# atenpas/gpd

Measured on AMD Instinct MI355X. Metric: 15-ch grasp candidates scored/sec (imagegen+LeNet) at 1/2/4/8 MI355X, higher is better.
Workload: dtype f64 geometry / u8 images / LeNet f32-equivalent by exact operand splitting: conv1 int8 digit planes of 32-bit fixed-point weights (i32 accumulate, exact), conv2 + ip1 three bf16 pieces per operand (six exact products per term, f32 accumulate), ip2 f32

## Files before the change

gpd_amd/csrc/gpd_internal.h:

```cpp
#pragma once
#include <hip/hip_runtime.h>
#include <stdint.h>

#include <cmath>

#include <vector>

#ifdef GPD_PROFILING
#include <cstdlib>
#include <rocprofiler-sdk-roctx/roctx.h>
#endif

#include "../../include/gpd_hip.h"

namespace gpd {

constexpr int kImg = 60;
constexpr int kPix = kImg * kImg;
constexpr int kFc1In = 7200;
constexpr int kFc1Out = 500;
__host__ __device__ inline size_t fc1p_index(int m, int kq, int u) { return (((size_t)(m >> 5) * 4 + kq) * kFc1Out + u) * 32 + (m & 31); }
constexpr int kLenetXld = 7296;

struct LeNetFast {
// ... 297 lines not shown
                 gpd_hand *d_out, hipStream_t stream);
int gather_records(const gpd_hand *d_all, const int32_t *d_sel, int k, gpd_hand *d_out, hipStream_t stream);
int select_topk_capacity();

struct ImageState {
  unsigned long long lcg_base = 0;
  int num_candidates = 0;
  int capacity = 0;
  uint8_t *d_images = nullptr;
  uint8_t *d_images_hwc = nullptr;
  uint32_t *d_set_bits = nullptr;
  int num_shadow_sets = 0, cap_shadow_sets = 0;
  bool wide = false;
  bool huge = false;
  int set_sd = 0, set_sr = 0;
  size_t cap_setwords = 0;
  int32_t *d_overflow2 = nullptr;
  char *d_huge_scratch = nullptr;
  int channels = 0;
  int slots = 0;
  int32_t *d_overflow = nullptr;
  int32_t *d_pts_overflow = nullptr;
  char *d_pts_scratch = nullptr;
  int32_t *d_status = nullptr;
  long long stat_sets = 0, stat_sum_set_ni = 0, stat_sum_cand_ni = 0;
  std::vector<unsigned char> consts;
  double view_points[3 * kMaxCams] = {0};
  hipStream_t aux = nullptr;
  hipEvent_t ev_fork = nullptr, ev_join = nullptr;
  bool side_stream = true;
};
int images_reserve(const gpd_params &p, ImageState &im, int n, int shadow_sets);
int images_run(const gpd_params &p, const Cloud &c, const SearchState &s, const Plan &pl, ImageState &im, hipStream_t stream);
int images_launch(const SearchState &s, const Plan &pl, ImageState &im, hipStream_t stream, bool counters_clean = false);
void images_status_text(int status, char *buf, size_t len);
int images_routes(const ImageState &im, int32_t *route, long long info[8]);
hipError_t planar_to_hwc(const uint8_t *src, uint8_t *dst, int n, int C, hipStream_t stream);
hipError_t hwc_to_planar(const uint8_t *src, uint8_t *dst, int n, int C, hipStream_t stream);
void image_cell_thresholds(double len, double *out);
void images_free(ImageState &im);

struct HostConsts {
  double rot[GPD_MAX_SLOTS][9];
  double rot_binormal[9];
  double finger_spacing[32];
  double deepen_depths[128];
// ... 46 lines not shown
```

gpd_amd/csrc/images.hip:

```cpp
#include <cfloat>
#include <cmath>
#include <cstddef>
#include <cstdio>
#include <cstdlib>
#include <cstring>

#include <mutex>
#include <type_traits>

#include "gpd_internal.h"

namespace gpd {

#define HIP_RET(expr)                                                                       \
  do {                                                                                      \
    hipError_t e_ = (expr);                                                                 \
    if (e_ != hipSuccess) {                                                                 \
      set_error("%s failed: %s (%s:%d)", #expr, hipGetErrorString(e_), __FILE__, __LINE__); \
      return GPD_ERR_HIP;                                                                   \
    }                                                                                       \
  } while (0)

constexpr int IMG_THREADS = 512;
constexpr int SET_THREADS = 1024;
// ... 3 lines not shown
constexpr int SH_CAP = 6144;
constexpr int SH_CAP_BIG = 12288;
template <bool WIDE>
struct Vox {
  static constexpr int VD = WIDE ? 64 : 46;
  static constexpr int SD = WIDE ? 128 : 86;
  static constexpr int SR = WIDE ? 64 : 43;
  static constexpr int LB = 18;
  static constexpr int SETWORDS = (SD * SD * SD + 31) / 32;
};

struct ImgConsts {
  double vol_depth, vol_width, vol_height, half_od, dbl_h;
  int C, nproj, per;
  double shadow_length, voxel, voxel_mult, rand_inv;
  int num_shadow;
  uint32_t stride_a, stride_c;
  double len[3];
  double inv_cell[3];
  double thr[3][kImg + 1];
  double inv_len[3];
  int true_div;
  int set_sd, set_sr;
};
__constant__ ImgConsts c_img;

struct ImgParams {
  const float *nn;
  int cap;
  const double *centers;
  const gpd_hand *hands;
  const int32_t *cand_hand;
  const int32_t *meta;
  const uint32_t *set_bits;
  uint8_t *images;
  int32_t *status;
  int num_cand;
  const int32_t *cand_list;
  const int32_t *cand_count;
  int32_t *overflow_list;
  int32_t *overflow_count;
  unsigned long long *dbg;
  int32_t *pts_overflow_list;
  int32_t *pts_overflow_count;
  char *pts_scratch;
  int exit_after;
  char *huge_scratch;
};

struct Box {
  double F[9];
  double sample[3];
  double off[3];
  double lo[3], hi[3];
};

constexpr size_t PTS_SCRATCH_BYTES = (size_t)PT_CAP_BIG * (3 * sizeof(double) + sizeof(float4) + sizeof(uint32_t));
struct PointArrays {
  double t[3][PT_CAP];
  float4 an[PT_CAP];
};
struct NoPointArrays {};
template <bool BIG>
struct __attribute__((aligned(16))) SmemPts {
  typename std::conditional<BIG, NoPointArrays, PointArrays>::type p;
  __attribute__((aligned(16))) uint32_t cells[kPix];
  uint16_t place[BIG ? PT_CAP_BIG : PT_CAP];
  float4 nzv[(BIG ? kPix : PT_CAP) + 1];
  uint16_t nzlist[BIG ? kPix : PT_CAP];
  double thr[3][kImg + 1];
  double recip[128];
  float red_f[4 * IMG_WAVES];
  int red_i[IMG_WAVES];
  int counter;
  int flag;
  int nnz;
};
typedef SmemPts<false> Smem;
template <int SHC, bool WIDE>
struct __attribute__((aligned(16))) SmemShadow {
  __attribute__((aligned(16))) float raster0[kPix];
  __attribute__((aligned(16))) uint32_t cells[kPix];
  uint32_t lin[SHC];
  union {
    struct {
      uint16_t rowbase[Vox<WIDE>::VD * Vox<WIDE>::VD];
      uint8_t rowcnt[Vox<WIDE>::VD * Vox<WIDE>::VD];
    } rows;
    uint16_t place[SHC];
  } bp;
  uint16_t nz[kPix];
  uint8_t cz[SHC];
  double thr[3][kImg + 1];
  double recip[128];
  float red_f[4 * IMG_WAVES];
  int red_i[IMG_WAVES];
  int vorg[3];
  int flag;
  int nnz;
};

__device__ inline double uniform_f64(double v) {
  const unsigned long long b = (unsigned long long)__double_as_longlong(v);
  const unsigned lo = __builtin_amdgcn_readfirstlane((unsigned)b);
  const unsigned hi = __builtin_amdgcn_readfirstlane((unsigned)(b >> 32));
  return __longlong_as_double((long long)(((unsigned long long)hi << 32) | lo));
}

template <class OP>
__device__ inline float wave_reduce_f32(float v, OP op) {
  auto dpp = [](float x, auto ctrl, auto rmask) {
    return __int_as_float(__builtin_amdgcn_update_dpp(__float_as_int(x), __float_as_int(x), decltype(ctrl)::value, decltype(rmask)::value, 0xf, false));
  };
  using std::integral_constant;
  v = op(v, dpp(v, integral_constant<int, 0xB1>(), integral_constant<int, 0xf>()));
  v = op(v, dpp(v, integral_constant<int, 0x4E>(), integral_constant<int, 0xf>()));
  v = op(v, dpp(v, integral_constant<int, 0x141>(), integral_constant<int, 0xf>()));
  v = op(v, dpp(v, integral_constant<int, 0x140>(), integral_constant<int, 0xf>()));
  v = op(v, dpp(v, integral_constant<int, 0x142>(), integral_constant<int, 0xa>()));
  v = op(v, dpp(v, integral_constant<int, 0x143>(), integral_constant<int, 0xc>()));
  return __int_as_float(__builtin_amdgcn_readlane(__float_as_int(v), 63));
}
__device__ inline float wave_max_f32(float v) { return wave_reduce_f32(v, [](float a, float b) { return fmaxf(a, b); }); }
__device__ inline float wave_min_f32(float v) { return wave_reduce_f32(v, [](float a, float b) { return fminf(a, b); }); }

__device__ inline int wave_incl_scan_i32(int v) {
  v += __builtin_amdgcn_update_dpp(0, v, 0x111, 0xf, 0xf, false);
  v += __builtin_amdgcn_update_dpp(0, v, 0x112, 0xf, 0xf, false);
  v += __builtin_amdgcn_update_dpp(0, v, 0x114, 0xf, 0xf, false);
  v += __builtin_amdgcn_update_dpp(0, v, 0x118, 0xf, 0xf, false);
// ... 457 lines not shown
#pragma unroll
      for (int i = 0; i < N; i++) {
        const int j = i ^ stride;
        if (j > i) {
          const uint32_t lo = min(k[i], k[j]), hi = max(k[i], k[j]);
          const bool up = (i & size) == 0;
          k[i] = up ? lo : hi;
          k[j] = up ? hi : lo;
        }
      }
    }
  }
}
template <int N>
__device__ inline void sort_u16_regs(uint16_t *p, int n) {
  uint32_t k[N];
#pragma unroll
  for (int q = 0; q < N; q++) k[q] = q < n ? (uint32_t)p[q] : 0xffffffffu;
  sort_regs<N>(k);
#pragma unroll
  for (int q = 0; q < N; q++)
    if (q < n) p[q] = (uint16_t)k[q];
}
#define TICK(k)                                                     \
  do {                                                              \
    if (P.dbg && tid == 0) {                                        \
      const unsigned long long now_ = __builtin_readcyclecounter(); \
      atomicAdd(&P.dbg[k], now_ - t_last);                          \
      t_last = now_;                                                \
    }                                                               \
  } while (0)

__device__ inline void load_box(const gpd_hand &H, Box &B) {
  const ImgConsts &K = c_img;
#pragma unroll
  for (int i = 0; i < 9; i++) B.F[i] = uniform_f64(H.frame[i]);
#pragma unroll
  for (int i = 0; i < 3; i++) B.sample[i] = uniform_f64(H.sample[i]);
  const double hb = uniform_f64(H.bottom), hc = uniform_f64(H.center);
  B.off[0] = hb;
  B.off[1] = uniform_f64(hc - K.half_od);
  B.off[2] = uniform_f64(-K.vol_height);
  B.lo[0] = hb;
  B.hi[0] = uniform_f64(hb + K.vol_depth);
  B.lo[1] = B.off[1];
  B.hi[1] = uniform_f64(hc + K.half_od);
  B.lo[2] = uniform_f64(-1.0 * K.vol_height);
  B.hi[2] = uniform_f64(K.vol_height);
}

__device__ __forceinline__ int xcd_candidate(int n) {
  const int per = (n + 7) >> 3;
  const int L = blockIdx.x, slot = L >> 3;
  const int cand = (L & 7) * per + slot;
  return cand < n ? cand : -1;
}

template <int SHC, bool WIDE>
__device__ __forceinline__ void shadow_image_body(const ImgParams &P, SmemShadow<SHC, WIDE> &S, const int cand) {
  constexpr int VDIM = Vox<WIDE>::VD, SD = Vox<WIDE>::SD, SR = Vox<WIDE>::SR, LB = Vox<WIDE>::LB, SETWORDS = Vox<WIDE>::SETWORDS;
  unsigned long long t_last = __builtin_readcyclecounter();
  const ImgConsts &K = c_img;
  const int tid = threadIdx.x;
  const int lane = tid & 63;
  const int set_ord = P.meta[4 * cand + 2];
  const int set_nb = P.meta[4 * cand + 3];
  uint8_t *out = P.images + (size_t)cand * kPix * K.C;
  Box B;
  load_box(P.hands[P.cand_hand[cand]], B);
  for (int i = tid; i < 3 * (kImg + 1); i += IMG_THREADS) (&S.thr[0][0])[i] = (&K.thr[0][0])[i];
  for (int i = tid; i < 128; i += IMG_THREADS) S.recip[i] = i ? 1.0 / (double)i : 0.0;
  for (int c = tid; c < kPix / 4; c += IMG_THREADS) reinterpret_cast<uint4 *>(S.cells)[c] = make_uint4(0u, 0u, 0u, 0u);
  if (tid == 0) {
    S.flag = 0;
    double lo[3] = {DBL_MAX, DBL_MAX, DBL_MAX}, hi[3] = {-DBL_MAX, -DBL_MAX, -DBL_MAX};
#pragma unroll
    for (int k = 0; k < 8; k++) {
      const double bx = (k & 1) ? B.hi[0] : B.lo[0];
      const double by = (k & 2) ? B.hi[1] : B.lo[1];
      const double bz = (k & 4) ? B.hi[2] : B.lo[2];
#pragma unroll
      for (int a = 0; a < 3; a++) {
        const double w = B.sample[a] + B.F[3 * a] * bx + B.F[3 * a + 1] * by + B.F[3 * a + 2] * bz;
        lo[a] = fmin(lo[a], w);
        hi[a] = fmax(hi[a], w);
      }
    }
    int bad = 0;
#pragma unroll
    for (int a = 0; a < 3; a++) {
      const int v0 = (int)floor(lo[a] * K.voxel_mult) - 1, v1 = (int)floor(hi[a] * K.voxel_mult) + 1;
      const int o = (int)floor(B.sample[a] * K.voxel_mult) - SR;
      S.vorg[a] = v0;
      if (v1 - v0 >= VDIM || v0 + 1 < o || v1 - 1 >= o + SD) bad = 1;
    }
    S.flag = bad;
  }
  __syncthreads();
  const int x0 = S.vorg[0], y0 = S.vorg[1], z0 = S.vorg[2];
  constexpr int NROWS = VDIM * VDIM, RPT = (NROWS + IMG_THREADS - 1) / IMG_THREADS;
  unsigned long long mask[RPT];
#pragma unroll
  for (int k = 0; k < RPT; k++) mask[k] = 0ull;
  if (set_ord >= 0) {
    const uint32_t *sb = P.set_bits + (size_t)set_ord * SETWORDS;
    const int ox = (int)floor(B.sample[0] * K.voxel_mult) - SR, oy = (int)floor(B.sample[1] * K.voxel_mult) - SR,
              oz = (int)floor(B.sample[2] * K.voxel_mult) - SR;
    const int zlo = z0 - oz;
    double invBz[3];
#pragma unroll
    for (int a = 0; a < 3; a++) {
      const double bz = B.F[6 + a] * K.voxel;
      invBz[a] = uniform_f64(fabs(bz) > 1e-9 ? 1.0 / bz : 0.0);
    }
    const int za = zlo < 0 ? 0 : zlo, zb = (zlo + VDIM < SD) ? zlo + VDIM : SD;
    const int nbits = zb - za;
    double T0[3], Ax[3], Ay[3], Lf[3], Wd[3];
    {
      const double wx = (double)x0 * K.voxel - B.sample[0], wy = (double)y0 * K.voxel - B.sample[1],
                   wz = (double)(za - zlo + z0) * K.voxel - B.sample[2];
#pragma unroll
      for (int a = 0; a < 3; a++) {
        T0[a] = uniform_f64(B.F[a] * wx + B.F[3 + a] * wy + B.F[6 + a] * wz);
        Ax[a] = uniform_f64(B.F[a] * K.voxel);
        Ay[a] = uniform_f64(B.F[3 + a] * K.voxel);
        Lf[a] = invBz[a] > 0.0 ? B.lo[a] : B.hi[a];
        Wd[a] = uniform_f64(fabs((B.hi[a] - B.lo[a]) * invBz[a]));
      }
    }
    unsigned long long fld[RPT];
#pragma unroll
    for (int k = 0; k < RPT; k++) fld[k] = 0ull;
    for (int cb = 0; cb < set_nb; cb++) {
      const uint32_t *sc = sb + (size_t)cb * SETWORDS;
      uint32_t wa[RPT], wb[RPT], wc[RPT];
#pragma unroll
      for (int k = 0; k < RPT; k++) {
        const int row = tid + k * IMG_THREADS;
        const int ix = row / VDIM, iy = row - ix * VDIM;
        const int sx = x0 + ix - ox, sy = y0 + iy - oy;
        const bool ok = row < NROWS && (unsigned)sx < (unsigned)SD && (unsigned)sy < (unsigned)SD && za < zb;
        const int w0 = ok ? ((sx * SD + sy) * SD + za) >> 5 : 0;
        wa[k] = sc[w0];
        wb[k] = sc[w0 + 1 < SETWORDS ? w0 + 1 : SETWORDS - 1];
        wc[k] = sc[w0 + 2 < SETWORDS ? w0 + 2 : SETWORDS - 1];
      }
#pragma unroll
      for (int k = 0; k < RPT; k++) {
        const int row = tid + k * IMG_THREADS;
        const int ix = row / VDIM, iy = row - ix * VDIM;
        const int sx = x0 + ix - ox, sy = y0 + iy - oy;
// ... 7 lines not shown
      }
    }
#pragma unroll
    for (int k = 0; k < RPT; k++) {
      const int row = tid + k * IMG_THREADS;
      if (row >= NROWS) continue;
      const int ix = row / VDIM, iy = row - ix * VDIM;
      unsigned long long field = fld[k];
      field &= (nbits >= 64) ? ~0ull : ((1ull << (nbits > 0 ? nbits : 0)) - 1ull);
      if (field) {
        constexpr double EPS = 1e-3;
        const double fx = (double)ix, fy = (double)iy;
        double dmin = 0.0, dmax = (double)(nbits - 1);
        double smin = 0.0, smax = (double)(nbits - 1);
#pragma unroll
        for (int a = 0; a < 3; a++) {
          const double tba = T0[a] + fx * Ax[a] + fy * Ay[a];
          if (invBz[a] != 0.0) {
            const double dl = (Lf[a] - tba) * invBz[a], dh = dl + Wd[a];
            dmin = fmax(dmin, dl - EPS);
            dmax = fmin(dmax, dh + EPS);
            smin = fmax(smin, dl + EPS);
            smax = fmin(smax, dh - EPS);
          } else if (tba < B.lo[a] - 1e-6 || tba > B.hi[a] + 1e-6) {
            dmax = -1.0;
          } else if (!(tba > B.lo[a] + 1e-6 && tba < B.hi[a] - 1e-6)) {
            smax = -1.0;
          }
        }
        if (dmax < dmin) {
          field = 0ull;
        } else {
          const int t0 = (int)ceil(dmin), t1 = (int)floor(dmax);
          if (t0 > 0) field &= ~((1ull << t0) - 1ull);
          if (t1 < 63) field &= (2ull << t1) - 1ull;
          if (smax >= smin) {
            const int u0 = (int)ceil(smin), u1 = (int)floor(smax);
            if (u1 >= u0) {
              unsigned long long sure = field;
              if (u0 > 0) sure &= ~((1ull << u0) - 1ull);
              if (u1 < 63) sure &= (2ull << u1) - 1ull;
              mask[k] |= sure << (za - zlo);
              field &= ~sure;
            }
          }
        }
      }
      while (field) {
        const int t = __ffsll((long long)field) - 1;
        field &= field - 1;
        const int iz = za + t - zlo;
        double th[3];
        to_hand(B, (double)(ix + x0) * K.voxel, (double)(iy + y0) * K.voxel, (double)(iz + z0) * K.voxel, th);
        if (in_box(B, th)) mask[k] |= 1ull << iz;
      }
    }
  }
#pragma unroll
  for (int k = 0; k < RPT; k++) {
    const int row = tid + k * IMG_THREADS;
    if (row < NROWS) S.bp.rows.rowcnt[row] = (uint8_t)__popcll(mask[k]);
  }
  __syncthreads();
  TICK(0);
  int cnt = 0;
#pragma unroll
  for (int k = 0; k < RPT; k++) {
    const int row = tid * RPT + k;
    if (row < NROWS) cnt += S.bp.rows.rowcnt[row];
  }
  int n_sh;
  int pos = block_excl_scan(S, cnt, &n_sh);
  if (n_sh > SHC) {
    if (tid == 0) {
      if (P.overflow_list) {
        const int slot = atomicAdd(P.overflow_count, 1);
        P.overflow_list[slot] = cand;
// ... 12 lines not shown
    }
  }
  __syncthreads();
#pragma unroll
  for (int k = 0; k < RPT; k++) {
    const int row = tid + k * IMG_THREADS;
    if (row >= NROWS) continue;
    unsigned long long m = mask[k];
    int at = S.bp.rows.rowbase[row];
    const int rx = row / VDIM, ry = row - rx * VDIM;
    const uint32_t rowpos = ((uint32_t)rx << 12) | ((uint32_t)ry << 6);
    while (m) {
      const int iz = __ffsll((long long)m) - 1;
      m &= m - 1;
      S.lin[at++] = rowpos | (uint32_t)iz;
    }
  }
  __syncthreads();
  const int ns = n_sh < SHC ? n_sh : SHC;
  if (P.dbg && tid == 0) {
    atomicMax(&P.dbg[28], (unsigned long long)n_sh);
    atomicAdd(&P.dbg[29], (unsigned long long)n_sh);
  }
  for (int k = tid; k < ns; k += IMG_THREADS) {
    const int lin = (int)S.lin[k];
    const int ix = lin >> 12, iy = (lin >> 6) & 63, iz = lin & 63;
    double th[3];
    to_hand(B, (double)(ix + x0) * K.voxel, (double)(iy + y0) * K.voxel, (double)(iz + z0) * K.voxel, th);
    const uint32_t c3 = cells_of(S, B, th);
    S.lin[k] = (uint32_t)lin | ((c3 & 0xfffu) << LB);
    S.cz[k] = (uint8_t)(c3 >> 12);
  }
  __syncthreads();
  TICK(1);
  auto cell_of_entry = [&](int k, int pr) {
    const uint32_t v = S.lin[k];
    return cell_of_key(((v >> LB) & 0xfffu) | ((uint32_t)S.cz[k] << 12), pr);
  };
  constexpr uint32_t EMPTY = 0xffffffffu;
  for (int pr = 0; pr < 3; pr++) {
    if (tid < 32) reinterpret_cast<int *>(S.red_f)[tid] = 0;
    for (int k = tid; k < ns; k += IMG_THREADS) atomicAdd(&S.cells[cell_of_entry(k, pr)], 1u);
    __syncthreads();
    uint32_t pk[2];
    scan_cells_hist(S, pk);
    scatter_nonempty(S, S.nz, pk);
// ... 45 lines not shown
    }
    __syncthreads();
    TICK(10);
    float gmax = -FLT_MAX;
    int gany = 0;
#pragma unroll
    for (int w = 0; w < IMG_WAVES; w++) {
      gmax = fmaxf(gmax, S.red_f[4 * w + 2]);
      gany |= reinterpret_cast<const int *>(S.red_f)[4 * w + 3];
    }
    const double mxd = gany ? (double)gmax : 0.0;
    const float mxf = (float)mxd;
    TICK(3);
    finalize_planes_ex<1, false>(
        S, &S.raster0[0], nullptr, out + (size_t)(pr * K.per + 4) * kPix,
        [mxf](float x) { return __float_as_uint(x) == EMPTY ? 0.0f - 0.0f : mxf - x; },
        [&S, tid] {
          int c0 = tid;
          asm volatile("" : "+v"(c0));
          for (int c = c0; c < kPix / 4; c += IMG_THREADS) reinterpret_cast<uint4 *>(S.cells)[c] = make_uint4(0u, 0u, 0u, 0u);
        });
    TICK(4);
  }
  if (tid == 0 && S.flag) atomicOr(P.status, S.flag);
}

constexpr int LGRID = 256;

template <int SHC, bool WIDE>
__global__ __launch_bounds__(IMG_THREADS, SHC <= SH_CAP ? 4 : 2) void shadow_image_kernel(ImgParams P) {
  __shared__ SmemShadow<SHC, WIDE> S;
  if constexpr (SHC > SH_CAP) {
    const int count = *P.cand_count;
    for (int q = blockIdx.x; q < count; q += gridDim.x) {
      __syncthreads();
      shadow_image_body<SHC, WIDE>(P, S, P.cand_list[q]);
    }
  } else {
    const int cand = xcd_candidate(P.num_cand);
    if (cand < 0) return;
    shadow_image_body<SHC, WIDE>(P, S, cand);
  }
}

constexpr int HUGE_CAP = 65535;
constexpr int HUGE_WIN = 256;
constexpr size_t HUGE_SCRATCH_BYTES = (size_t)HUGE_WIN * HUGE_WIN * sizeof(int32_t) + (size_t)(HUGE_CAP + 1) * (2 * sizeof(uint32_t) + sizeof(uint16_t)) + 64;
struct __attribute__((aligned(16))) SmemAny {
  __attribute__((aligned(16))) float raster0[kPix];
  __attribute__((aligned(16))) uint32_t cells[kPix];
  uint16_t nz[kPix];
  double thr[3][kImg + 1];
  double recip[128];
  float red_f[4 * IMG_WAVES];
  int red_i[IMG_WAVES];
  int vorg[3], wdim[3];
  int flag;
};

__device__ void shadow_image_any_body(const ImgParams &P, SmemAny &S, const int cand, char *scratch) {
  const ImgConsts &K = c_img;
  const int SD = K.set_sd, SR = K.set_sr;
  const size_t SETWORDS = (size_t)(((long long)SD * SD * SD + 31) / 32);
  const int tid = threadIdx.x;
  const int lane = tid & 63;
  const int set_ord = P.meta[4 * cand + 2];
  const int set_nb = P.meta[4 * cand + 3];
  uint8_t *out = P.images + (size_t)cand * kPix * K.C;
  int32_t *rowtab = reinterpret_cast<int32_t *>(scratch);
  uint32_t *lin = reinterpret_cast<uint32_t *>(rowtab + HUGE_WIN * HUGE_WIN);
  uint32_t *ckey = lin + (HUGE_CAP + 1);
  uint16_t *place = reinterpret_cast<uint16_t *>(ckey + (HUGE_CAP + 1));
  Box B;
  load_box(P.hands[P.cand_hand[cand]], B);
  for (int i = tid; i < 3 * (kImg + 1); i += IMG_THREADS) (&S.thr[0][0])[i] = (&K.thr[0][0])[i];
  for (int i = tid; i < 128; i += IMG_THREADS) S.recip[i] = i ? 1.0 / (double)i : 0.0;
  if (tid == 0) {
    double lo[3] = {DBL_MAX, DBL_MAX, DBL_MAX}, hi[3] = {-DBL_MAX, -DBL_MAX, -DBL_MAX};
    for (int k = 0; k < 8; k++) {
      const double bx = (k & 1) ? B.hi[0] : B.lo[0];
      const double by = (k & 2) ? B.hi[1] : B.lo[1];
      const double bz = (k & 4) ? B.hi[2] : B.lo[2];
      for (int a = 0; a < 3; a++) {
        const double w = B.sample[a] + B.F[3 * a] * bx + B.F[3 * a + 1] * by + B.F[3 * a + 2] * bz;
        lo[a] = fmin(lo[a], w);
        hi[a] = fmax(hi[a], w);
      }
    }
    int bad = 0;
    for (int a = 0; a < 3; a++) {
      const int v0 = (int)floor(lo[a] * K.voxel_mult) - 1, v1 = (int)floor(hi[a] * K.voxel_mult) + 1;
      const int o = (int)floor(B.sample[a] * K.voxel_mult) - SR;
      S.vorg[a] = v0;
      S.wdim[a] = v1 - v0 + 1;
      if (v1 - v0 + 1 > HUGE_WIN || v0 + 1 < o || v1 - 1 >= o + SD) bad = 1;
    }
    S.flag = bad;
  }
  __syncthreads();
  if (S.flag) {
    if (tid == 0) atomicOr(P.status, 1);
    return;
  }
  const int x0 = S.vorg[0], y0 = S.vorg[1], z0 = S.vorg[2];
  const int wx = S.wdim[0], wy = S.wdim[1], wz = S.wdim[2];
  const int nrows = wx * wy;
  const int ox = (int)floor(B.sample[0] * K.voxel_mult) - SR, oy = (int)floor(B.sample[1] * K.voxel_mult) - SR,
            oz = (int)floor(B.sample[2] * K.voxel_mult) - SR;
  auto walk_row = [&](int row, auto emit) {
    const int ix = row / wy, iy = row - ix * wy;
    const int sx = x0 + ix - ox, sy = y0 + iy - oy;
    if (set_ord < 0 || (unsigned)sx >= (unsigned)SD || (unsigned)sy >= (unsigned)SD) return;
    const int zlo = z0 - oz;
    const int za = zlo < 0 ? 0 : zlo, zb = zlo + wz < SD ? zlo + wz : SD;
    if (za >= zb) return;
    const long long rowbit = ((long long)sx * SD + sy) * SD;
    for (long long w = (rowbit + za) >> 5; w <= (rowbit + zb - 1) >> 5; w++) {
      uint32_t bits = ~0u;
      for (int cb = 0; cb < set_nb; cb++) bits &= P.set_bits[((size_t)set_ord + cb) * SETWORDS + (size_t)w];
      const long long first = w << 5;
      if (first < rowbit + za) bits &= ~0u << (int)(rowbit + za - first);
      if (first + 32 > rowbit + zb) bits &= ~0u >> (int)(first + 32 - (rowbit + zb));
      while (bits) {
        const int t = __ffs((int)bits) - 1;
        bits &= bits - 1;
        const int iz = (int)(first + t - rowbit) - zlo;
        double th[3];
        to_hand(B, (double)(ix + x0) * K.voxel, (double)(iy + y0) * K.voxel, (double)(iz + z0) * K.voxel, th);
        if (in_box(B, th)) emit(iz);
      }
    }
// ... 99 lines not shown
    }
    const double mxd = gany ? (double)gmax : 0.0;
    const float mxf = (float)mxd;
    __syncthreads();
    for (int c = tid; c < kPix; c += IMG_THREADS) S.raster0[c] = ((S.cells[c] & 0xffffu) ? mxf : 0.0f) - S.raster0[c];
    __syncthreads();
    finalize_planes<1>(S, &S.raster0[0], nullptr, out + (size_t)(pr * K.per + 4) * kPix);
  }
}

__global__ __launch_bounds__(IMG_THREADS) void shadow_image_any_kernel(ImgParams P) {
  __shared__ SmemAny S;
  char *scratch = P.huge_scratch + (size_t)blockIdx.x * HUGE_SCRATCH_BYTES;
  const int count = P.cand_list ? *P.cand_count : P.num_cand;
  for (int q = blockIdx.x; q < count; q += gridDim.x) {
    __syncthreads();
    shadow_image_any_body(P, S, P.cand_list ? P.cand_list[q] : q, scratch);
  }
}

template <bool BIG>
__device__ __forceinline__ void grasp_image_body(const ImgParams &P, SmemPts<BIG> &S, const int cand) {
  constexpr int CAP = BIG ? PT_CAP_BIG : PT_CAP;
  unsigned long long t_last = __builtin_readcyclecounter();
  const ImgConsts &K = c_img;
  const int tid = threadIdx.x;
  const int lane = tid & 63;
  const int slot_s = P.meta[4 * cand + 0];
  const int N = P.meta[4 * cand + 1];
  const float *nn = P.nn + (size_t)slot_s * 6 * P.cap;
  uint8_t *out = P.images + (size_t)cand * kPix * K.C;
  double *gt = nullptr;
  float4 *gan = nullptr;
  uint32_t *gidx = nullptr;
  if constexpr (BIG) {
    char *row = P.pts_scratch + (size_t)blockIdx.x * PTS_SCRATCH_BYTES;
    gt = reinterpret_cast<double *>(row);
    gan = reinterpret_cast<float4 *>(row + (size_t)CAP * 3 * sizeof(double));
    gidx = reinterpret_cast<uint32_t *>(row + (size_t)CAP * (3 * sizeof(double) + sizeof(float4)));
  }
  auto IDX = [&](int e) -> int {
    if constexpr (BIG) return (int)gidx[e];
    else return (int)S.place[e];
  };
  auto T = [&](int a, int e) -> double & {
    if constexpr (BIG) return gt[(size_t)a * CAP + e];
    else return S.p.t[a][e];
  };
  auto AN = [&](int e) -> float4 & {
    if constexpr (BIG) return gan[e];
    else return S.p.an[e];
  };
  Box B;
  load_box(P.hands[P.cand_hand[cand]], B);
  for (int i = tid; i < 3 * (kImg + 1); i += IMG_THREADS) (&S.thr[0][0])[i] = (&K.thr[0][0])[i];
  for (int i = tid; i < 128; i += IMG_THREADS) S.recip[i] = i ? 1.0 / (double)i : 0.0;
  if (tid == 0) {
    S.flag = 0;
    S.nzv[0] = make_float4(0.f, 0.f, 0.f, 0.f);
  }
  for (int c = tid; c < kPix / 4; c += IMG_THREADS) reinterpret_cast<uint4 *>(S.cells)[c] = make_uint4(0u, 0u, 0u, 0u);
  __syncthreads();
  int n_before = 0;
  static_assert(offsetof(SmemPts<BIG>, nzlist) % sizeof(int) == 0 && sizeof(S.nzlist) >= 16 * IMG_WAVES * sizeof(int), "ballot counts in nzlist");
  int *cnt = reinterpret_cast<int *>(S.nzlist);
  constexpr int RB = 16;
  const int wave = tid >> 6;
  for (int b0 = 0; b0 < N; b0 += RB * IMG_THREADS) {
    unsigned inmask = 0;
    const int left = N - b0, nr = left >= RB * IMG_THREADS ? RB : (left + IMG_THREADS - 1) / IMG_THREADS;
    for (int r0 = 0; r0 < nr; r0 += 4) {
      float px[4], py[4], pz[4];
#pragma unroll
      for (int q = 0; q < 4; q++) {
        const int i = b0 + (r0 + q) * IMG_THREADS + tid;
        const int ic = i < N ? i : N - 1;
        px[q] = nn[0 * P.cap + ic];
        py[q] = nn[1 * P.cap + ic];
        pz[q] = nn[2 * P.cap + ic];
// ... 442 lines not shown
  double top = len * 2.0;
  std::memcpy(&hi, &top, sizeof(hi));
  while (hi - lo > 1) {
    const uint64_t mid = lo + (hi - lo) / 2;
    double x;
    std::memcpy(&x, &mid, sizeof(x));
    if (f(x))
      hi = mid;
    else
      lo = mid;
  }
  double x;
  std::memcpy(&x, &hi, sizeof(x));
  return x;
}

void image_cell_thresholds(double len, double *out) {
  out[0] = 0.0;
  for (int k = 1; k < kImg; k++) out[k] = cell_threshold(len, k);
  out[kImg] = DBL_MAX;
}

void images_free(ImageState &im) {
  void *ptrs[] = {im.d_images, im.d_images_hwc, im.d_status, im.d_set_bits, im.d_overflow, im.d_overflow2, im.d_pts_overflow, im.d_pts_scratch, im.d_huge_scratch};
  for (void *p : ptrs)
    if (p) (void)hipFree(p);
  if (im.ev_fork) (void)hipEventDestroy(im.ev_fork);
  if (im.ev_join) (void)hipEventDestroy(im.ev_join);
  if (im.aux) (void)hipStreamDestroy(im.aux);
  im = ImageState();
}

int images_reserve(const gpd_params &p, ImageState &im, int n, int shadow_sets) {
  const int C = p.image_num_channels;
  if (!im.d_status) {
    HIP_RET(hipMalloc(&im.d_status, 4 * sizeof(int32_t)));
    HIP_RET(hipMemset(im.d_status, 0, 4 * sizeof(int32_t)));
    HIP_RET(hipMalloc(&im.d_pts_scratch, (size_t)LGRID * PTS_SCRATCH_BYTES));
  }
  if (n > im.capacity) {
    note_alloc(__func__);
    void *ptrs[] = {im.d_images, im.d_images_hwc, im.d_overflow, im.d_overflow2, im.d_pts_overflow};
    for (void *q : ptrs)
      if (q) (void)hipFree(q);
    im.d_overflow = nullptr;
    im.d_overflow2 = nullptr;
    im.d_pts_overflow = nullptr;
    im.d_images = nullptr;
    im.d_images_hwc = nullptr;
    im.capacity = 0;
    const int cap = n + n / 4;
    HIP_RET(hipMalloc(&im.d_images, (size_t)cap * kPix * C));
    HIP_RET(hipMalloc(&im.d_overflow, (size_t)cap * sizeof(int32_t)));
    HIP_RET(hipMalloc(&im.d_overflow2, (size_t)cap * sizeof(int32_t)));
    HIP_RET(hipMalloc(&im.d_pts_overflow, (size_t)cap * sizeof(int32_t)));
    im.capacity = cap;
  }
  {
    const double vox = 0.003;
    const double diag = std::sqrt(p.volume_depth * p.volume_depth + p.volume_width * p.volume_width + 4.0 * p.volume_height * p.volume_height);
    const double rx = std::fmax(p.hand_depth - p.init_bite, p.volume_depth);
    const double ry = 0.5 * (p.hand_outer_diameter - p.finger_width) + 0.5 * p.volume_width;
    const double reach = std::sqrt(rx * rx + ry * ry + p.volume_height * p.volume_height);
    const double need_win = std::ceil(diag / vox) + 3.0, need_reach = std::ceil(reach / vox) + 1.0;
    im.wide = need_win > (double)Vox<false>::VD || need_reach > (double)(Vox<false>::SR - 1);
    im.huge = need_win > (double)Vox<true>::VD || need_reach > (double)(Vox<true>::SR - 1);
    if (im.huge) {
      if (need_reach + 2.0 > 640.0) {
        set_error("images: an image volume with %.2f m of reach is beyond the shadow region this library allocates", reach);
        return GPD_ERR_CAPACITY;
      }
      im.set_sr = (int)need_reach + 2;
      im.set_sd = 2 * im.set_sr;
    } else {
      im.set_sr = im.wide ? Vox<true>::SR : Vox<false>::SR;
      im.set_sd = im.wide ? Vox<true>::SD : Vox<false>::SD;
    }
  }
// ... 37 lines not shown
  HIP_RET(hipMemsetAsync(im.d_status, 0, 4 * sizeof(int32_t), stream));
  if (n == 0) return GPD_OK;
  ImgConsts k;
  std::memset(&k, 0, sizeof(k));
  k.vol_depth = p.volume_depth;
  k.vol_width = p.volume_width;
  k.vol_height = p.volume_height;
  k.half_od = p.volume_width / 2.0;
  k.dbl_h = 2.0 * p.volume_height;
  k.C = C;
  k.nproj = (C <= 3) ? 1 : 3;
  k.per = (C == 15) ? 5 : (C == 12 ? 4 : C);
  k.shadow_length = std::fmax(std::fmax(p.volume_depth, p.volume_height / 2.0), p.volume_width);
  k.voxel = 0.003;
  k.voxel_mult = 1.0 / 0.003;
  k.rand_inv = 1.0 / 32767.0;
  k.num_shadow = (int)std::floor(k.shadow_length / k.voxel);
  k.len[0] = k.vol_depth;
  k.len[1] = k.vol_width;
  k.len[2] = k.dbl_h;
  k.true_div = 0;
  k.set_sd = im.set_sd;
  k.set_sr = im.set_sr;
  {
    struct AxisCache {
      double len = -1.0, thr[kImg + 1], inv_len = 0.0;
      int true_div = 0;
    };
    static AxisCache cache[3];
    static std::mutex cache_mutex;
    std::lock_guard<std::mutex> lock(cache_mutex);
    for (int a = 0; a < 3; a++) {
      AxisCache &ac = cache[a];
      if (ac.len != k.len[a]) {
        ac.len = k.len[a];
        image_cell_thresholds(k.len[a], ac.thr);
        ac.inv_len = 1.0 / k.len[a];
        ac.true_div = 0;
        uint64_t rs = 88172645463325252ull;
        for (int i = 0; i < 200000 && !ac.true_div; i++) {
          rs ^= rs << 13;
          rs ^= rs >> 7;
          rs ^= rs << 17;
          double x = (double)(rs >> 11) * (1.0 / 9007199254740992.0) * k.len[a];
          if (i & 1) x = (double)(float)x;
          if (i < kImg) x = ac.thr[i];
// ... 41 lines not shown
  HIP_RET(hipMemcpyToSymbolAsync(HIP_SYMBOL(c_img), want.data(), sizeof(ImgConsts), 0, hipMemcpyHostToDevice, stream));
  HIP_RET(hipStreamSynchronize(stream));
  loaded = want;
  return GPD_OK;
}

int images_launch(const SearchState &s, const Plan &pl, ImageState &im, hipStream_t stream, bool counters_clean) {
  const int n = im.num_candidates;
  if (n <= 0) return GPD_OK;
  if (!counters_clean) HIP_RET(hipMemsetAsync(im.d_status + 1, 0, 3 * sizeof(int32_t), stream));
  std::lock_guard<std::mutex> consts_lock(g_img_mutex);
  {
    const int rc = load_img_consts(im.consts, stream);
    if (rc) return rc;
  }
  ImgParams ip;
  std::memset(&ip, 0, sizeof(ip));
  ip.nn = s.d_nn;
  ip.cap = s.nn_cap;
  ip.centers = s.d_centers;
  ip.hands = s.d_hands;
  ip.cand_hand = pl.d_cand_hand;
  ip.meta = pl.d_cand_meta;
  ip.images = im.d_images;
  ip.status = im.d_status;
  static unsigned long long *d_dbg = nullptr;
  ip.dbg = nullptr;
  ip.exit_after = prof_env("GPD_IMG_EXIT") ? atoi(prof_env("GPD_IMG_EXIT")) : 0;
  if (prof_env("GPD_IMG_TIMING")) {
    if (!d_dbg) HIP_RET(hipMalloc(&d_dbg, 32 * sizeof(unsigned long long)));
    HIP_RET(hipMemsetAsync(d_dbg, 0, 32 * sizeof(unsigned long long), stream));
    ip.dbg = d_dbg;
  }
  ip.set_bits = im.d_set_bits;
  ip.cand_list = nullptr;
  ip.cand_count = nullptr;
  ip.num_cand = n;
  ip.overflow_list = nullptr;
  ip.overflow_count = nullptr;
  if (!im.aux) {
    HIP_RET(hipStreamCreate(&im.aux));
    HIP_RET(hipEventCreateWithFlags(&im.ev_fork, hipEventDisableTiming));
    HIP_RET(hipEventCreateWithFlags(&im.ev_join, hipEventDisableTiming));
  }
  static const bool serial = prof_env("GPD_IMG_SERIAL") != nullptr;
  static const size_t lds_pad = prof_env("GPD_IMG_LDS_PAD") ? (size_t)atoi(prof_env("GPD_IMG_LDS_PAD")) : 0;
  hipStream_t pts_stream = (im.channels == 15 && !ip.dbg && im.side_stream && !serial) ? im.aux : stream;
  if (pts_stream != stream) {
    HIP_RET(hipEventRecord(im.ev_fork, stream));
    HIP_RET(hipStreamWaitEvent(pts_stream, im.ev_fork, 0));
  }
  ip.pts_overflow_list = im.d_pts_overflow;
  ip.pts_overflow_count = im.d_status + 3;
  ip.pts_scratch = nullptr;
  grasp_image_kernel<false><<<8 * ((n + 7) / 8), IMG_THREADS, lds_pad, pts_stream>>>(ip);
  HIP_RET(hipGetLastError());
  {
    ImgParams ib = ip;
    ib.cand_list = im.d_pts_overflow;
    ib.cand_count = im.d_status + 3;
    ib.pts_overflow_list = nullptr;
    ib.pts_overflow_count = nullptr;
    ib.pts_scratch = im.d_pts_scratch;
    grasp_image_kernel<true><<<LGRID, IMG_THREADS, 0, pts_stream>>>(ib);
    HIP_RET(hipGetLastError());
  }
  ip.pts_overflow_list = nullptr;
  ip.pts_overflow_count = nullptr;
  if (im.num_shadow_sets > 0) {
    SetParams sp;
// ... 126 lines not shown
```

Measured before the change: 2.164 million.

## Precompute per-candidate box geometry in a separate kernel and read via scalar loads

Adds a small cand_box_kernel that computes each candidate's hand frame, voxel window, bounds flag and row-walk constants once into a global CandBox array. The image kernels then read these through constant-address-space scalar loads instead of recomputing them on thread 0 followed by __syncthreads. The reciprocal table moves into constant memory, and the profiling tick counters compile out when profiling is off. The cost is an extra kernel launch and global traffic per candidate, plus repeated scalar reloads of box fields inside the inner loops.

```diff
diff --git a/gpd_amd/csrc/gpd_internal.h b/gpd_amd/csrc/gpd_internal.h
--- a/gpd_amd/csrc/gpd_internal.h
+++ b/gpd_amd/csrc/gpd_internal.h
@@ -343,6 +343,7 @@
   int32_t *d_overflow = nullptr;
   int32_t *d_pts_overflow = nullptr;
   char *d_pts_scratch = nullptr;
+  void *d_cand_box = nullptr;
   int32_t *d_status = nullptr;
   long long stat_sets = 0, stat_sum_set_ni = 0, stat_sum_cand_ni = 0;
   std::vector<unsigned char> consts;
diff --git a/gpd_amd/csrc/images.hip b/gpd_amd/csrc/images.hip
--- a/gpd_amd/csrc/images.hip
+++ b/gpd_amd/csrc/images.hip
@@ -49,10 +49,13 @@
   double inv_len[3];
   int true_div;
   int set_sd, set_sr;
+  double recip[128];
 };
 __constant__ ImgConsts c_img;
 
+struct CandBox;
 struct ImgParams {
+  const CandBox *cbox;
   const float *nn;
   int cap;
   const double *centers;
@@ -81,6 +84,18 @@
   double off[3];
   double lo[3], hi[3];
 };
+struct __attribute__((aligned(16))) CandBox {
+  Box B;
+  double invBz[3], T0[3], Ax[3], Ay[3], Lf[3], Wd[3];
+  int32_t meta[4];
+  int32_t vorg[3];
+  int32_t bad_region;
+  int32_t ext[3];
+  int32_t pad0;
+  int32_t org[3];
+  int32_t pad1;
+};
+static_assert(sizeof(CandBox) % 16 == 0, "CandBox rows stay 16-byte aligned");
 
 constexpr size_t PTS_SCRATCH_BYTES = (size_t)PT_CAP_BIG * (3 * sizeof(double) + sizeof(float4) + sizeof(uint32_t));
 struct PointArrays {
@@ -122,8 +137,6 @@
   double recip[128];
   float red_f[4 * IMG_WAVES];
   int red_i[IMG_WAVES];
-  int vorg[3];
-  int flag;
   int nnz;
 };
 
@@ -133,6 +146,7 @@
   const unsigned hi = __builtin_amdgcn_readfirstlane((unsigned)(b >> 32));
   return __longlong_as_double((long long)(((unsigned long long)hi << 32) | lo));
 }
+__device__ inline int uniform_i32(int v) { return __builtin_amdgcn_readfirstlane(v); }
 
 template <class OP>
 __device__ inline float wave_reduce_f32(float v, OP op) {
@@ -636,6 +650,8 @@
   for (int q = 0; q < N; q++)
     if (q < n) p[q] = (uint16_t)k[q];
 }
+#ifdef GPD_PROFILING
+#define TICK_START() __builtin_readcyclecounter()
 #define TICK(k)                                                     \
   do {                                                              \
     if (P.dbg && tid == 0) {                                        \
@@ -644,23 +660,108 @@
       t_last = now_;                                                \
     }                                                               \
   } while (0)
+#else
+#define TICK_START() 0ull
+#define TICK(k) \
+  do {          \
+  } while (0)
+#endif
 
 __device__ inline void load_box(const gpd_hand &H, Box &B) {
   const ImgConsts &K = c_img;
 #pragma unroll
-  for (int i = 0; i < 9; i++) B.F[i] = uniform_f64(H.frame[i]);
-#pragma unroll
-  for (int i = 0; i < 3; i++) B.sample[i] = uniform_f64(H.sample[i]);
-  const double hb = uniform_f64(H.bottom), hc = uniform_f64(H.center);
+  for (int i = 0; i < 9; i++) B.F[i] = H.frame[i];
+#pragma unroll
+  for (int i = 0; i < 3; i++) B.sample[i] = H.sample[i];
+  const double hb = H.bottom, hc = H.center;
   B.off[0] = hb;
-  B.off[1] = uniform_f64(hc - K.half_od);
-  B.off[2] = uniform_f64(-K.vol_height);
+  B.off[1] = hc - K.half_od;
+  B.off[2] = -K.vol_height;
   B.lo[0] = hb;
-  B.hi[0] = uniform_f64(hb + K.vol_depth);
+  B.hi[0] = hb + K.vol_depth;
   B.lo[1] = B.off[1];
-  B.hi[1] = uniform_f64(hc + K.half_od);
-  B.lo[2] = uniform_f64(-1.0 * K.vol_height);
-  B.hi[2] = uniform_f64(K.vol_height);
+  B.hi[1] = hc + K.half_od;
+  B.lo[2] = -1.0 * K.vol_height;
+  B.hi[2] = K.vol_height;
+}
+__device__ inline void box_window(const Box &B, int SR, int SD, CandBox &R) {
+  const ImgConsts &K = c_img;
+  double lo[3] = {DBL_MAX, DBL_MAX, DBL_MAX}, hi[3] = {-DBL_MAX, -DBL_MAX, -DBL_MAX};
+#pragma unroll
+  for (int k = 0; k < 8; k++) {
+    const double bx = (k & 1) ? B.hi[0] : B.lo[0];
+    const double by = (k & 2) ? B.hi[1] : B.lo[1];
+    const double bz = (k & 4) ? B.hi[2] : B.lo[2];
+#pragma unroll
+    for (int a = 0; a < 3; a++) {
+      const double w = B.sample[a] + B.F[3 * a] * bx + B.F[3 * a + 1] * by + B.F[3 * a + 2] * bz;
+      lo[a] = fmin(lo[a], w);
+      hi[a] = fmax(hi[a], w);
+    }
+  }
+  int bad = 0;
+#pragma unroll
+  for (int a = 0; a < 3; a++) {
+    const int v0 = (int)floor(lo[a] * K.voxel_mult) - 1, v1 = (int)floor(hi[a] * K.voxel_mult) + 1;
+    const int o = (int)floor(B.sample[a] * K.voxel_mult) - SR;
+    R.vorg[a] = v0;
+    R.ext[a] = v1 - v0;
+    R.org[a] = o;
+    if (v0 + 1 < o || v1 - 1 >= o + SD) bad = 1;
+  }
+  R.bad_region = bad;
+}
+__device__ inline void row_constants(const Box &B, CandBox &R) {
+  const ImgConsts &K = c_img;
+  const int x0 = R.vorg[0], y0 = R.vorg[1], z0 = R.vorg[2];
+  const int zlo = z0 - R.org[2];
+  const int za = zlo < 0 ? 0 : zlo;
+#pragma unroll
+  for (int a = 0; a < 3; a++) {
+    const double bz = B.F[6 + a] * K.voxel;
+    R.invBz[a] = fabs(bz) > 1e-9 ? 1.0 / bz : 0.0;
+  }
+  const double wx = (double)x0 * K.voxel - B.sample[0], wy = (double)y0 * K.voxel - B.sample[1],
+               wz = (double)(za - zlo + z0) * K.voxel - B.sample[2];
+#pragma unroll
+  for (int a = 0; a < 3; a++) {
+    R.T0[a] = B.F[a] * wx + B.F[3 + a] * wy + B.F[6 + a] * wz;
+    R.Ax[a] = B.F[a] * K.voxel;
+    R.Ay[a] = B.F[3 + a] * K.voxel;
+    R.Lf[a] = R.invBz[a] > 0.0 ? B.lo[a] : B.hi[a];
+    R.Wd[a] = fabs((B.hi[a] - B.lo[a]) * R.invBz[a]);
+  }
+}
+constexpr int CBOX_THREADS = 128;
+__global__ __launch_bounds__(CBOX_THREADS) void cand_box_kernel(const gpd_hand *__restrict__ hands, const int32_t *__restrict__ cand_hand,
+                                                                const int32_t *__restrict__ meta, CandBox *__restrict__ out, int n, int sr, int sd) {
+  const int cand = blockIdx.x * CBOX_THREADS + threadIdx.x;
+  if (cand >= n) return;
+  CandBox R;
+  load_box(hands[cand_hand[cand]], R.B);
+#pragma unroll
+  for (int w = 0; w < 4; w++) R.meta[w] = meta[4 * cand + w];
+  box_window(R.B, sr, sd, R);
+  row_constants(R.B, R);
+  R.pad0 = R.pad1 = 0;
+  out[cand] = R;
+}
+__device__ __forceinline__ const CandBox &at_use(const CandBox &R) {
+  const unsigned long long a = (unsigned long long)&R;
+  unsigned lo = __builtin_amdgcn_readfirstlane((unsigned)a), hi = __builtin_amdgcn_readfirstlane((unsigned)(a >> 32));
+  asm volatile("" : "+s"(lo), "+s"(hi));
+  typedef const CandBox __attribute__((address_space(4))) *ConstPtr;
+  return *(const CandBox *)(ConstPtr)(((unsigned long long)hi << 32) | lo);
+}
+__device__ __forceinline__ void read_box(const CandBox &R, Box &B) {
+#pragma unroll
+  for (int i = 0; i < 9; i++) B.F[i] = uniform_f64(R.B.F[i]);
+#pragma unroll
+  for (int i = 0; i < 3; i++) {
+    B.sample[i] = uniform_f64(R.B.sample[i]);
+    B.off[i] = B.lo[i] = uniform_f64(R.B.lo[i]);
+    B.hi[i] = uniform_f64(R.B.hi[i]);
+  }
 }
 
 __device__ __forceinline__ int xcd_candidate(int n) {
@@ -672,75 +773,39 @@
 
 template <int SHC, bool WIDE>
 __device__ __forceinline__ void shadow_image_body(const ImgParams &P, SmemShadow<SHC, WIDE> &S, const int cand) {
-  constexpr int VDIM = Vox<WIDE>::VD, SD = Vox<WIDE>::SD, SR = Vox<WIDE>::SR, LB = Vox<WIDE>::LB, SETWORDS = Vox<WIDE>::SETWORDS;
-  unsigned long long t_last = __builtin_readcyclecounter();
+  constexpr int VDIM = Vox<WIDE>::VD, SD = Vox<WIDE>::SD, LB = Vox<WIDE>::LB, SETWORDS = Vox<WIDE>::SETWORDS;
+  [[maybe_unused]] unsigned long long t_last = TICK_START();
   const ImgConsts &K = c_img;
   const int tid = threadIdx.x;
   const int lane = tid & 63;
-  const int set_ord = P.meta[4 * cand + 2];
-  const int set_nb = P.meta[4 * cand + 3];
+  const CandBox &R = at_use(P.cbox[cand]);
+  const int set_ord = uniform_i32(R.meta[2]);
+  const int set_nb = uniform_i32(R.meta[3]);
   uint8_t *out = P.images + (size_t)cand * kPix * K.C;
-  Box B;
-  load_box(P.hands[P.cand_hand[cand]], B);
   for (int i = tid; i < 3 * (kImg + 1); i += IMG_THREADS) (&S.thr[0][0])[i] = (&K.thr[0][0])[i];
-  for (int i = tid; i < 128; i += IMG_THREADS) S.recip[i] = i ? 1.0 / (double)i : 0.0;
+  for (int i = tid; i < 128; i += IMG_THREADS) S.recip[i] = K.recip[i];
   for (int c = tid; c < kPix / 4; c += IMG_THREADS) reinterpret_cast<uint4 *>(S.cells)[c] = make_uint4(0u, 0u, 0u, 0u);
-  if (tid == 0) {
-    S.flag = 0;
-    double lo[3] = {DBL_MAX, DBL_MAX, DBL_MAX}, hi[3] = {-DBL_MAX, -DBL_MAX, -DBL_MAX};
-#pragma unroll
-    for (int k = 0; k < 8; k++) {
-      const double bx = (k & 1) ? B.hi[0] : B.lo[0];
-      const double by = (k & 2) ? B.hi[1] : B.lo[1];
-      const double bz = (k & 4) ? B.hi[2] : B.lo[2];
-#pragma unroll
-      for (int a = 0; a < 3; a++) {
-        const double w = B.sample[a] + B.F[3 * a] * bx + B.F[3 * a + 1] * by + B.F[3 * a + 2] * bz;
-        lo[a] = fmin(lo[a], w);
-        hi[a] = fmax(hi[a], w);
-      }
-    }
-    int bad = 0;
-#pragma unroll
-    for (int a = 0; a < 3; a++) {
-      const int v0 = (int)floor(lo[a] * K.voxel_mult) - 1, v1 = (int)floor(hi[a] * K.voxel_mult) + 1;
-      const int o = (int)floor(B.sample[a] * K.voxel_mult) - SR;
-      S.vorg[a] = v0;
-      if (v1 - v0 >= VDIM || v0 + 1 < o || v1 - 1 >= o + SD) bad = 1;
-    }
-    S.flag = bad;
-  }
-  __syncthreads();
-  const int x0 = S.vorg[0], y0 = S.vorg[1], z0 = S.vorg[2];
+  const int x0 = uniform_i32(R.vorg[0]), y0 = uniform_i32(R.vorg[1]), z0 = uniform_i32(R.vorg[2]);
   constexpr int NROWS = VDIM * VDIM, RPT = (NROWS + IMG_THREADS - 1) / IMG_THREADS;
   unsigned long long mask[RPT];
 #pragma unroll
   for (int k = 0; k < RPT; k++) mask[k] = 0ull;
   if (set_ord >= 0) {
     const uint32_t *sb = P.set_bits + (size_t)set_ord * SETWORDS;
-    const int ox = (int)floor(B.sample[0] * K.voxel_mult) - SR, oy = (int)floor(B.sample[1] * K.voxel_mult) - SR,
-              oz = (int)floor(B.sample[2] * K.voxel_mult) - SR;
+    const CandBox &Rr = at_use(R);
+    const int ox = uniform_i32(Rr.org[0]), oy = uniform_i32(Rr.org[1]), oz = uniform_i32(Rr.org[2]);
     const int zlo = z0 - oz;
-    double invBz[3];
-#pragma unroll
-    for (int a = 0; a < 3; a++) {
-      const double bz = B.F[6 + a] * K.voxel;
-      invBz[a] = uniform_f64(fabs(bz) > 1e-9 ? 1.0 / bz : 0.0);
-    }
     const int za = zlo < 0 ? 0 : zlo, zb = (zlo + VDIM < SD) ? zlo + VDIM : SD;
     const int nbits = zb - za;
-    double T0[3], Ax[3], Ay[3], Lf[3], Wd[3];
-    {
-      const double wx = (double)x0 * K.voxel - B.sample[0], wy = (double)y0 * K.voxel - B.sample[1],
-                   wz = (double)(za - zlo + z0) * K.voxel - B.sample[2];
-#pragma unroll
-      for (int a = 0; a < 3; a++) {
-        T0[a] = uniform_f64(B.F[a] * wx + B.F[3 + a] * wy + B.F[6 + a] * wz);
-        Ax[a] = uniform_f64(B.F[a] * K.voxel);
-        Ay[a] = uniform_f64(B.F[3 + a] * K.voxel);
-        Lf[a] = invBz[a] > 0.0 ? B.lo[a] : B.hi[a];
-        Wd[a] = uniform_f64(fabs((B.hi[a] - B.lo[a]) * invBz[a]));
-      }
+    double invBz[3], T0[3], Ax[3], Ay[3], Lf[3], Wd[3];
+#pragma unroll
+    for (int a = 0; a < 3; a++) {
+      invBz[a] = uniform_f64(Rr.invBz[a]);
+      T0[a] = uniform_f64(Rr.T0[a]);
+      Ax[a] = uniform_f64(Rr.Ax[a]);
+      Ay[a] = uniform_f64(Rr.Ay[a]);
+      Lf[a] = uniform_f64(Rr.Lf[a]);
+      Wd[a] = uniform_f64(Rr.Wd[a]);
     }
     unsigned long long fld[RPT];
 #pragma unroll
@@ -794,10 +859,13 @@
             dmax = fmin(dmax, dh + EPS);
             smin = fmax(smin, dl + EPS);
             smax = fmin(smax, dh - EPS);
-          } else if (tba < B.lo[a] - 1e-6 || tba > B.hi[a] + 1e-6) {
-            dmax = -1.0;
-          } else if (!(tba > B.lo[a] + 1e-6 && tba < B.hi[a] - 1e-6)) {
-            smax = -1.0;
+          } else {
+            const double blo = uniform_f64(Rr.B.lo[a]), bhi = uniform_f64(Rr.B.hi[a]);
+            if (tba < blo - 1e-6 || tba > bhi + 1e-6) {
+              dmax = -1.0;
+            } else if (!(tba > blo + 1e-6 && tba < bhi - 1e-6)) {
+              smax = -1.0;
+            }
           }
         }
         if (dmax < dmin) {
@@ -822,9 +890,11 @@
         const int t = __ffsll((long long)field) - 1;
         field &= field - 1;
         const int iz = za + t - zlo;
+        Box Bx;
+        read_box(at_use(R), Bx);
         double th[3];
-        to_hand(B, (double)(ix + x0) * K.voxel, (double)(iy + y0) * K.voxel, (double)(iz + z0) * K.voxel, th);
-        if (in_box(B, th)) mask[k] |= 1ull << iz;
+        to_hand(Bx, (double)(ix + x0) * K.voxel, (double)(iy + y0) * K.voxel, (double)(iz + z0) * K.voxel, th);
+        if (in_box(Bx, th)) mask[k] |= 1ull << iz;
       }
     }
   }
@@ -883,6 +953,8 @@
     atomicMax(&P.dbg[28], (unsigned long long)n_sh);
     atomicAdd(&P.dbg[29], (unsigned long long)n_sh);
   }
+  Box B;
+  read_box(at_use(R), B);
   for (int k = tid; k < ns; k += IMG_THREADS) {
     const int lin = (int)S.lin[k];
     const int ix = lin >> 12, iy = (lin >> 6) & 63, iz = lin & 63;
@@ -974,7 +1046,7 @@
         });
     TICK(4);
   }
-  if (tid == 0 && S.flag) atomicOr(P.status, S.flag);
+  if (tid == 0 && (R.bad_region | (R.ext[0] >= VDIM) | (R.ext[1] >= VDIM) | (R.ext[2] >= VDIM))) atomicOr(P.status, 1);
 }
 
 constexpr int LGRID = 256;
@@ -1006,59 +1078,35 @@
   double recip[128];
   float red_f[4 * IMG_WAVES];
   int red_i[IMG_WAVES];
-  int vorg[3], wdim[3];
-  int flag;
 };
 
 __device__ void shadow_image_any_body(const ImgParams &P, SmemAny &S, const int cand, char *scratch) {
   const ImgConsts &K = c_img;
-  const int SD = K.set_sd, SR = K.set_sr;
+  const int SD = K.set_sd;
   const size_t SETWORDS = (size_t)(((long long)SD * SD * SD + 31) / 32);
   const int tid = threadIdx.x;
   const int lane = tid & 63;
-  const int set_ord = P.meta[4 * cand + 2];
-  const int set_nb = P.meta[4 * cand + 3];
+  const CandBox &R = at_use(P.cbox[cand]);
+  const int set_ord = uniform_i32(R.meta[2]);
+  const int set_nb = uniform_i32(R.meta[3]);
   uint8_t *out = P.images + (size_t)cand * kPix * K.C;
   int32_t *rowtab = reinterpret_cast<int32_t *>(scratch);
   uint32_t *lin = reinterpret_cast<uint32_t *>(rowtab + HUGE_WIN * HUGE_WIN);
   uint32_t *ckey = lin + (HUGE_CAP + 1);
   uint16_t *place = reinterpret_cast<uint16_t *>(ckey + (HUGE_CAP + 1));
   Box B;
-  load_box(P.hands[P.cand_hand[cand]], B);
+  read_box(R, B);
   for (int i = tid; i < 3 * (kImg + 1); i += IMG_THREADS) (&S.thr[0][0])[i] = (&K.thr[0][0])[i];
-  for (int i = tid; i < 128; i += IMG_THREADS) S.recip[i] = i ? 1.0 / (double)i : 0.0;
-  if (tid == 0) {
-    double lo[3] = {DBL_MAX, DBL_MAX, DBL_MAX}, hi[3] = {-DBL_MAX, -DBL_MAX, -DBL_MAX};
-    for (int k = 0; k < 8; k++) {
-      const double bx = (k & 1) ? B.hi[0] : B.lo[0];
-      const double by = (k & 2) ? B.hi[1] : B.lo[1];
-      const double bz = (k & 4) ? B.hi[2] : B.lo[2];
-      for (int a = 0; a < 3; a++) {
-        const double w = B.sample[a] + B.F[3 * a] * bx + B.F[3 * a + 1] * by + B.F[3 * a + 2] * bz;
-        lo[a] = fmin(lo[a], w);
-        hi[a] = fmax(hi[a], w);
-      }
-    }
-    int bad = 0;
-    for (int a = 0; a < 3; a++) {
-      const int v0 = (int)floor(lo[a] * K.voxel_mult) - 1, v1 = (int)floor(hi[a] * K.voxel_mult) + 1;
-      const int o = (int)floor(B.sample[a] * K.voxel_mult) - SR;
-      S.vorg[a] = v0;
-      S.wdim[a] = v1 - v0 + 1;
-      if (v1 - v0 + 1 > HUGE_WIN || v0 + 1 < o || v1 - 1 >= o + SD) bad = 1;
-    }
-    S.flag = bad;
-  }
-  __syncthreads();
-  if (S.flag) {
+  for (int i = tid; i < 128; i += IMG_THREADS) S.recip[i] = K.recip[i];
+  const int x0 = uniform_i32(R.vorg[0]), y0 = uniform_i32(R.vorg[1]), z0 = uniform_i32(R.vorg[2]);
+  const int wx = uniform_i32(R.ext[0]) + 1, wy = uniform_i32(R.ext[1]) + 1, wz = uniform_i32(R.ext[2]) + 1;
+  if (uniform_i32(R.bad_region) || wx > HUGE_WIN || wy > HUGE_WIN || wz > HUGE_WIN) {
     if (tid == 0) atomicOr(P.status, 1);
     return;
   }
-  const int x0 = S.vorg[0], y0 = S.vorg[1], z0 = S.vorg[2];
-  const int wx = S.wdim[0], wy = S.wdim[1], wz = S.wdim[2];
+  __syncthreads();
   const int nrows = wx * wy;
-  const int ox = (int)floor(B.sample[0] * K.voxel_mult) - SR, oy = (int)floor(B.sample[1] * K.voxel_mult) - SR,
-            oz = (int)floor(B.sample[2] * K.voxel_mult) - SR;
+  const int ox = uniform_i32(R.org[0]), oy = uniform_i32(R.org[1]), oz = uniform_i32(R.org[2]);
   auto walk_row = [&](int row, auto emit) {
     const int ix = row / wy, iy = row - ix * wy;
     const int sx = x0 + ix - ox, sy = y0 + iy - oy;
@@ -1204,12 +1252,13 @@
 template <bool BIG>
 __device__ __forceinline__ void grasp_image_body(const ImgParams &P, SmemPts<BIG> &S, const int cand) {
   constexpr int CAP = BIG ? PT_CAP_BIG : PT_CAP;
-  unsigned long long t_last = __builtin_readcyclecounter();
+  [[maybe_unused]] unsigned long long t_last = TICK_START();
   const ImgConsts &K = c_img;
   const int tid = threadIdx.x;
   const int lane = tid & 63;
-  const int slot_s = P.meta[4 * cand + 0];
-  const int N = P.meta[4 * cand + 1];
+  const CandBox &R = at_use(P.cbox[cand]);
+  const int slot_s = uniform_i32(R.meta[0]);
+  const int N = uniform_i32(R.meta[1]);
   const float *nn = P.nn + (size_t)slot_s * 6 * P.cap;
   uint8_t *out = P.images + (size_t)cand * kPix * K.C;
   double *gt = nullptr;
@@ -1234,9 +1283,9 @@
     else return S.p.an[e];
   };
   Box B;
-  load_box(P.hands[P.cand_hand[cand]], B);
+  read_box(R, B);
   for (int i = tid; i < 3 * (kImg + 1); i += IMG_THREADS) (&S.thr[0][0])[i] = (&K.thr[0][0])[i];
-  for (int i = tid; i < 128; i += IMG_THREADS) S.recip[i] = i ? 1.0 / (double)i : 0.0;
+  for (int i = tid; i < 128; i += IMG_THREADS) S.recip[i] = K.recip[i];
   if (tid == 0) {
     S.flag = 0;
     S.nzv[0] = make_float4(0.f, 0.f, 0.f, 0.f);
@@ -1725,7 +1774,7 @@
 }
 
 void images_free(ImageState &im) {
-  void *ptrs[] = {im.d_images, im.d_images_hwc, im.d_status, im.d_set_bits, im.d_overflow, im.d_overflow2, im.d_pts_overflow, im.d_pts_scratch, im.d_huge_scratch};
+  void *ptrs[] = {im.d_images, im.d_images_hwc, im.d_status, im.d_set_bits, im.d_overflow, im.d_overflow2, im.d_pts_overflow, im.d_pts_scratch, im.d_huge_scratch, im.d_cand_box};
   for (void *p : ptrs)
     if (p) (void)hipFree(p);
   if (im.ev_fork) (void)hipEventDestroy(im.ev_fork);
@@ -1743,9 +1792,10 @@
   }
   if (n > im.capacity) {
     note_alloc(__func__);
-    void *ptrs[] = {im.d_images, im.d_images_hwc, im.d_overflow, im.d_overflow2, im.d_pts_overflow};
+    void *ptrs[] = {im.d_images, im.d_images_hwc, im.d_overflow, im.d_overflow2, im.d_pts_overflow, im.d_cand_box};
     for (void *q : ptrs)
       if (q) (void)hipFree(q);
+    im.d_cand_box = nullptr;
     im.d_overflow = nullptr;
     im.d_overflow2 = nullptr;
     im.d_pts_overflow = nullptr;
@@ -1757,6 +1807,7 @@
     HIP_RET(hipMalloc(&im.d_overflow, (size_t)cap * sizeof(int32_t)));
     HIP_RET(hipMalloc(&im.d_overflow2, (size_t)cap * sizeof(int32_t)));
     HIP_RET(hipMalloc(&im.d_pts_overflow, (size_t)cap * sizeof(int32_t)));
+    HIP_RET(hipMalloc(&im.d_cand_box, (size_t)cap * sizeof(CandBox)));
     im.capacity = cap;
   }
   {
@@ -1840,6 +1891,7 @@
   k.true_div = 0;
   k.set_sd = im.set_sd;
   k.set_sr = im.set_sr;
+  for (int i = 1; i < 128; i++) k.recip[i] = 1.0 / (double)i;
   {
     struct AxisCache {
       double len = -1.0, thr[kImg + 1], inv_len = 0.0;
@@ -1927,6 +1979,7 @@
   ip.hands = s.d_hands;
   ip.cand_hand = pl.d_cand_hand;
   ip.meta = pl.d_cand_meta;
+  ip.cbox = static_cast<const CandBox *>(im.d_cand_box);
   ip.images = im.d_images;
   ip.status = im.d_status;
   static unsigned long long *d_dbg = nullptr;
@@ -1951,6 +2004,9 @@
   static const bool serial = prof_env("GPD_IMG_SERIAL") != nullptr;
   static const size_t lds_pad = prof_env("GPD_IMG_LDS_PAD") ? (size_t)atoi(prof_env("GPD_IMG_LDS_PAD")) : 0;
   hipStream_t pts_stream = (im.channels == 15 && !ip.dbg && im.side_stream && !serial) ? im.aux : stream;
+  cand_box_kernel<<<(n + CBOX_THREADS - 1) / CBOX_THREADS, CBOX_THREADS, 0, stream>>>(s.d_hands, pl.d_cand_hand, pl.d_cand_meta,
+                                                                                     static_cast<CandBox *>(im.d_cand_box), n, im.set_sr, im.set_sd);
+  HIP_RET(hipGetLastError());
   if (pts_stream != stream) {
     HIP_RET(hipEventRecord(im.ev_fork, stream));
     HIP_RET(hipStreamWaitEvent(pts_stream, im.ev_fork, 0));
```

New measurement: 2.154 million. No clear change (-0.4%).
